# researchmm/MM-Diffusion

Hardware: AMD Instinct MI355X
Metric: denoising steps/sec (video+audio pair), 16x64x64 / 25600 (higher is better)
Workload: dtype bf16; 1 GPU; BASELINE configs[1]: Landscape base model (133.68M params), DDPM p_sample, timestep_respacing=250, per-GPU batch 4, 16x3x64x64 video + 1x25600 audio; global_batch=4, parallelism=batch-sharded x1, no in-loop collective, weights=key-seeded synthetic (mm_diffusion.synth), graph_replay=True, batch_lanes=2, finite=True, ranks_seen=1

## Files before the change

### include/mmd.h

```cpp
#ifndef MMD_H
#define MMD_H
#include <stdint.h>
#ifdef __cplusplus
extern "C" {
#endif

#define MMD_F32 0
#define MMD_BF16 1
#define MMD_OK 0
#define MMD_ERR_ARG (-1)
#define MMD_ERR_LAUNCH (-2)
#define MMD_ERR_UNSUPPORTED (-3)

int mmd_version(void);
const char* mmd_last_error(void);
int mmd_debug_install_crash_handler(void);

int mmd_graph_begin(void* stream);
int mmd_graph_end(void* stream, void** exec_out);
int mmd_graph_launch(void* exec, void* stream);
int mmd_graph_destroy(void* exec);
int mmd_stream_create(void** stream_out);
int mmd_stream_sync(void* stream);
int mmd_stream_destroy(void* stream);
int mmd_event_create(void** ev);
int mmd_event_record(void* ev, void* stream);
int mmd_stream_wait_event(void* stream, void* ev);
int mmd_event_elapsed_ms(void* ev_start, void* ev_stop, float* ms);
int mmd_event_destroy(void* ev);

int mmd_temb_fwd(const void* t, int t_kind, int N, int dim, const float* W0, const float* b0, const float* W2,
                 const float* b2, float* out_silu, float* out_raw, void* stream);

int mmd_linear_fwd(const float* x, const float* W, const float* b, float* y, int N, int K, int J, void* stream);

int64_t mmd_gn_workspace_bytes(int dtype, int C, int S, int Tn);
int mmd_gn_stats(int dtype, const void* x, int64_t ld, int C, int S, int Tn, int inner, int64_t outer_stride,
                 int64_t inner_stride, int64_t tstride, const float* gamma, const float* beta, const float* film,
                 int64_t film_ld, float eps, float* a_out, float* b_out, float* mr_out, void* workspace, void* stream);
int mmd_gn_finalize_stats(const float* rec, int64_t rec_ld, int C, int S, int Tn, const float* gamma, const float* beta,
                          const float* film, int64_t film_ld, float eps, float* a_out, float* b_out, float* mr_out, void* stream);
int mmd_gn_apply(int dtype, const void* x, int64_t ldx, void* y, int64_t ldy, int64_t rows, int C, int S, int Tn, int inner,
                 int64_t outer_stride, int64_t inner_stride, int64_t tstride, const float* a, const float* b, int act,
                 void* stream);
int mmd_add_rowbias(int dtype, void* x, int64_t ld, int64_t rows, int C, int64_t rows_per_sample, const float* e,
                    int64_t e_ld, void* stream);
int mmd_colsum_slices(int dtype, const void* dY, int64_t lddy, int S, int64_t Tn, int C, float* out, int64_t ldo, void* stream);

int mmd_conv_gemm(int dtype, const void* A, int64_t lda, const void* W, const float* bias, const void* R, int64_t ldr,
                  void* Y, int64_t ldy, int M, int Cout, int Cin, int ntaps, const int* taps, int D0, int D1, int D2, int tile,
                  void* stream);

int mmd_gn_conv1x1(int dtype, const void* A, int64_t lda, const float* gn_a, const float* gn_b, int act, int S,
                   int64_t rows_per_slice, const void* W, const float* bias, const void* R, int64_t ldr, void* Y, int64_t ldy,
                   int M, int Cout, int Cin, int tile, void* stream);

int mmd_gn_small(int dtype, const void* x, int64_t ldx, void* y, int64_t ldy, int C, int S, int Tn, int inner, int64_t outer_stride,
                 int64_t inner_stride, int64_t tstride, const float* gamma, const float* beta, float eps, int act, void* stream);

int mmd_gn_group(int dtype, const void* x, int64_t ldx, void* y, int64_t ldy, int C, int S, int Tn, int inner, int64_t outer_stride,
                 int64_t inner_stride, int64_t tstride, const float* gamma, const float* beta, const float* film, int64_t film_ld,
                 float eps, int act, float* a_out, float* b_out, float* mr_out, void* stream);

int mmd_zero(void* ptr, int64_t bytes, void* stream);

int mmd_conv_gemm_stats(int dtype, const void* A, int64_t lda, const void* W, const float* bias, const void* R, int64_t ldr,
                        void* Y, int64_t ldy, int M, int Cout, int Cin, int ntaps, const int* taps, int D0, int D1, int D2, int tile,
                        float* stats, int64_t stats_ld, void* stream);
int mmd_gn_conv1x1_stats(int dtype, const void* A, int64_t lda, const float* gn_a, const float* gn_b, int act, int S,
                         int64_t rows_per_slice, const void* W, const float* bias, const void* R, int64_t ldr, void* Y, int64_t ldy,
                         int M, int Cout, int Cin, int tile, float* stats, int64_t stats_ld, void* stream);

int mmd_gn_conv1x1_skip(int dtype, const void* h, int64_t ldh, const float* gn_a, const float* gn_b, int act, int S,
                        int64_t rows_per_slice, const void* W_out, const float* bias_out, const void* x, int64_t ldx, int K2,
                        const void* W_skip, const float* bias_skip, void* Y, int64_t ldy, int M, int Cout, int K1, float* stats,
                        int64_t stats_ld, void* stream);

// ... 184 lines not shown
```

### mm-diffusion_amd/csrc/mmd_norm.hip

```cpp
#include "mmd_common.h"

#define GN_GROUPS 32
typedef __attribute__((ext_vector_type(2))) double f64x2;

struct SliceGeom {
  int S, Tn, inner;
  int64_t outer_stride, inner_stride, tstride;
};

__device__ __forceinline__ int64_t slice_base(const SliceGeom& g, int s) {
  return (int64_t)(s / g.inner) * g.outer_stride + (int64_t)(s % g.inner) * g.inner_stride;
}
__device__ __forceinline__ int slice_of_row(const SliceGeom& g, int64_t m) {
  const int64_t o = m / g.outer_stride, rem = m % g.outer_stride;
  return (int)(o * g.inner + (rem / g.inner_stride) % g.inner);
}

template <typename T, bool ONE>
__global__ __launch_bounds__(256) void gn_partial_kernel(const char* __restrict__ x, int64_t ld, int C, SliceGeom g, int R,
                                                         double* __restrict__ part, int nchunks,
                                                         const float* __restrict__ gamma, const float* __restrict__ beta,
                                                         const float* __restrict__ film, int64_t film_ld, float eps,
                                                         float* __restrict__ a_out, float* __restrict__ b_out, float* __restrict__ mr_out) {
  constexpr int EPV = Elt<T>::EPV;
// ... 149 lines not shown
    }
    s_pa[cl][gi] = (a[0] + a[1]) + (a[2] + a[3]);
    s_pb[cl][gi] = (b[0] + b[1]) + (b[2] + b[3]);
  }
  __syncthreads();
  if (tid < GN_GROUPS) {
    double a = 0.0, b = 0.0;
    for (int k = 0; k < 32; ++k) { a += s_pa[k][tid]; b += s_pb[k][tid]; }
    const double cnt = (double)Tn * (double)cpg;
    const double dm = a / cnt;
    double var = b / cnt - dm * dm;
    if (var < 0.0) var = 0.0;
    s_mean[tid] = (float)(piv + dm);
    s_rstd[tid] = (float)(1.0 / sqrt(var + (double)eps));
    if (mr_out) {
      mr_out[((int64_t)s * GN_GROUPS + tid) * 2] = s_mean[tid];
      mr_out[((int64_t)s * GN_GROUPS + tid) * 2 + 1] = s_rstd[tid];
    }
  }
  __syncthreads();
#pragma unroll
  for (int k = 0; k < CPT; ++k) {
    const int c = tid + k * 1024;
    if (c < C) {
      const int gi = c / cpg;
      const float a = s_rstd[gi] * gm[k];
      const float b = bt[k] - s_mean[gi] * a;
      a_out[(int64_t)s * C + c] = a * fsc[k];
      b_out[(int64_t)s * C + c] = b * fsc[k] + fsh[k];
    }
  }
}

template <typename T>
__global__ __launch_bounds__(256) void gn_apply_kernel(const char* __restrict__ x, int64_t ldx, char* __restrict__ y, int64_t ldy,
                                                       int C, SliceGeom g, const float* __restrict__ a,
                                                       const float* __restrict__ b, int act, int R) {
  constexpr int EPV = Elt<T>::EPV;
  constexpr int ES = 16 / EPV;
  const int s = blockIdx.y, chunk = blockIdx.x, tid = threadIdx.x;
  const int CV = C / EPV, CVB = min(CV, 256), RPP = 256 / CVB;
  const int col0 = tid % CVB, rl = tid / CVB;
  if (rl >= RPP) return;
  for (int cp = 0; cp < CV; cp += 256) {
  const int col = col0 + cp;
  if (col >= CV) break;
  float av[EPV], bv[EPV];
#pragma unroll
  for (int e = 0; e < EPV; e += 4) {
    const f32x4 a4 = *(const f32x4*)(a + (int64_t)s * C + col * EPV + e), b4 = *(const f32x4*)(b + (int64_t)s * C + col * EPV + e);
#pragma unroll
    for (int k = 0; k < 4; ++k) { av[e + k] = a4[k]; bv[e + k] = b4[k]; }
  }
  const int64_t base = slice_base(g, s);
  const char* xp = x + (base * ldx + (int64_t)col * EPV) * ES;
  char* yp = y + (base * ldy + (int64_t)col * EPV) * ES;
  const int64_t xs = g.tstride * ldx * ES, ys = g.tstride * ldy * ES;
  const int j0 = chunk * R, j1 = min(j0 + R, g.Tn);
  for (int jb = j0 + rl; jb < j1; jb += 4 * RPP) {
    u32x4 v[4];
#pragma unroll
    for (int u = 0; u < 4; ++u) {
      const int j = jb + u * RPP;
      if (j < j1) v[u] = *(const u32x4*)(xp + (int64_t)j * xs);
    }
#pragma unroll
    for (int u = 0; u < 4; ++u) {
      const int j = jb + u * RPP;
      if (j < j1) {
        float f[EPV];
        Elt<T>::unpack(v[u], f);
#pragma unroll
        for (int e = 0; e < EPV; ++e) {
          const float w = f[e] * av[e] + bv[e];
          f[e] = act ? silu_f(w) : w;
        }
        *(u32x4*)(yp + (int64_t)j * ys) = Elt<T>::pack(f);
      }
    }
  }
  }
}

template <typename T>
__global__ __launch_bounds__(256) void gn_small_kernel(const char* __restrict__ x, int64_t ldx, char* __restrict__ y, int64_t ldy, int C,
                                                       SliceGeom g, const float* __restrict__ gamma, const float* __restrict__ beta,
                                                       float eps, int act, int SPB) {
  constexpr int EPV = Elt<T>::EPV, ES = 16 / EPV, MAXT = 16, QPV = EPV / 4;
  extern __shared__ __attribute__((aligned(16))) char smem[];
  float* sQ = (float*)smem;
  const int CV = C / EPV, NQ = C / 4, cpg = C / GN_GROUPS, qpg = cpg / 4;
  const int tid = threadIdx.x, pl = tid / CV, cv = tid - pl * CV;
  const int s = blockIdx.x * SPB + pl;
  const bool live = pl < SPB && s < g.S;
  u32x4 v[MAXT];
  const int64_t base = live ? slice_base(g, s) : 0;
  const char* xp = x + (base * ldx + (int64_t)cv * EPV) * ES;
  const int64_t xs = g.tstride * ldx * ES;
#pragma unroll
  for (int j = 0; j < MAXT; ++j)
    if (live && j < g.Tn) v[j] = *(const u32x4*)(xp + (int64_t)j * xs);
  float q[2] = {0.f, 0.f};
  if (live) {
#pragma unroll
    for (int j = 0; j < MAXT; ++j)
      if (j < g.Tn) {
        float f[EPV];
        Elt<T>::unpack(v[j], f);
#pragma unroll
// ... 103 lines not shown
  if (C <= 0 || S <= 0 || Tn <= 0) return 0;
  return (int64_t)S * cdiv(Tn, gn_rows_per_block(dtype, C, S, Tn)) * GN_GROUPS * 2 * sizeof(double);
}

extern "C" int mmd_gn_stats(int dtype, const void* x, int64_t ld, int C, int S, int Tn, int inner, int64_t outer_stride,
                            int64_t inner_stride, int64_t tstride, const float* gamma, const float* beta,
                            const float* film, int64_t film_ld, float eps, float* a_out, float* b_out, float* mr_out,
                            void* workspace, void* stream) {
  int rc = check_geom("gn_stats", dtype, C, S, Tn, inner);
  if (rc) return rc;
  MMD_REQUIRE(x && gamma && beta && a_out && b_out, "gn_stats: null pointer");
  MMD_REQUIRE(((uintptr_t)x) % 16 == 0 && ld % (dtype == MMD_BF16 ? 8 : 4) == 0, "gn_stats: x must be 16-byte aligned rows");
  SliceGeom g{S, Tn, inner, outer_stride, inner_stride, tstride};
  hipStream_t st = (hipStream_t)stream;
  const int R = gn_rows_per_block(dtype, C, S, Tn);
  const int nchunks = cdiv(Tn, R);
  if (nchunks == 1)
    return mmd_by_dtype(dtype, [&](auto t) {
      return mmd_launch<gn_partial_kernel<typename decltype(t)::type, true>>("gn_stats_one", dim3(1, S), dim3(256), 0, st, (const char*)x, ld, C, g, R,
                                                                             (double*)nullptr, 1, gamma, beta, film, film_ld, eps, a_out, b_out, mr_out);
    });
  MMD_REQUIRE(workspace && ((uintptr_t)workspace) % 16 == 0, "gn_stats: 16-byte aligned workspace required for multi-block slices");
  dim3 grid(nchunks, S);
  rc = mmd_by_dtype(dtype, [&](auto t) {
    return mmd_launch<gn_partial_kernel<typename decltype(t)::type, false>>("gn_partial", grid, dim3(256), 0, st, (const char*)x, ld, C, g, R,
                                                                            (double*)workspace, nchunks, gamma, beta, film, film_ld, eps, a_out, b_out,
                                                                            (float*)nullptr);
  });
  if (rc) return rc;
  return mmd_launch<gn_finalize_kernel>("gn_finalize", dim3(S), dim3(1024), 0, st, (const char*)x, dtype, ld, g, (const double*)workspace, nchunks, C, Tn,
                                        gamma, beta, film, film_ld, eps, a_out, b_out, mr_out);
}

__global__ __launch_bounds__(256) void gn_finalize_rec_kernel(const float* __restrict__ rec, int64_t rec_ld, int C, int S, int Tn,
                                                              const float* __restrict__ gamma, const float* __restrict__ beta,
                                                              const float* __restrict__ film, int64_t film_ld, float eps,
                                                              float* __restrict__ a_out, float* __restrict__ b_out, float* __restrict__ mr_out) {
  __shared__ double s_a[4], s_b[4];
  const int gi = blockIdx.x, s = blockIdx.y, tid = threadIdx.x;
  const int cpg = C / GN_GROUPS, qpg = cpg / 4;
  const int nrec = Tn / 64;
  const float* base = rec + ((int64_t)s * nrec * rec_ld + (int64_t)gi * qpg) * 2;
  const int total = nrec * qpg;
  const int c = gi * cpg + min(tid, cpg - 1);
  const float gv = gamma[c], bv0 = beta[c];
  float fsc = 0.f, fsh = 0.f;
  if (film) {
    fsc = film[(int64_t)s * film_ld + c];
    fsh = film[(int64_t)s * film_ld + C + c];
  }
  double a[4] = {0.0, 0.0, 0.0, 0.0}, b[4] = {0.0, 0.0, 0.0, 0.0};
  for (int i = tid; i < total; i += 1024) {
#pragma unroll
    for (int u = 0; u < 4; ++u) {
      const int k = i + 256 * u;
      const int kk = min(k, total - 1);
      const int r = kk / qpg, cq = kk - r * qpg;
      const float2 v = *(const float2*)(base + ((int64_t)r * rec_ld + cq) * 2);
      const double m = k < total ? 1.0 : 0.0;
      a[u] += m * (double)v.x;
      b[u] += m * (double)v.y;
    }
  }
  double ta = (a[0] + a[1]) + (a[2] + a[3]), tb = (b[0] + b[1]) + (b[2] + b[3]);
  ta = wave_sum_d(ta);
  tb = wave_sum_d(tb);
  if ((tid & 63) == 0) { s_a[tid >> 6] = ta; s_b[tid >> 6] = tb; }
  __syncthreads();
  if (tid < cpg) {
    const double sa = (s_a[0] + s_a[1]) + (s_a[2] + s_a[3]), sb = (s_b[0] + s_b[1]) + (s_b[2] + s_b[3]);
    const double cnt = (double)Tn * (double)cpg;
    const double mean = sa / cnt;
    double var = sb / cnt - mean * mean;
    if (var < 0.0) var = 0.0;
    const float mean_f = (float)mean, rstd_f = (float)(1.0 / sqrt(var + (double)eps));
    if (mr_out && tid == 0) {
      mr_out[((int64_t)s * GN_GROUPS + gi) * 2] = mean_f;
      mr_out[((int64_t)s * GN_GROUPS + gi) * 2 + 1] = rstd_f;
    }
    float av = rstd_f * gv;
    float bv = bv0 - mean_f * av;
    if (film) {
      const float sc = 1.f + fsc;
      av *= sc;
      bv = bv * sc + fsh;
    }
    a_out[(int64_t)s * C + c] = av;
    b_out[(int64_t)s * C + c] = bv;
  }
}

extern "C" int mmd_gn_finalize_stats(const float* rec, int64_t rec_ld, int C, int S, int Tn, const float* gamma, const float* beta,
                                     const float* film, int64_t film_ld, float eps, float* a_out, float* b_out, float* mr_out,
                                     void* stream) {
  MMD_REQUIRE(rec && gamma && beta && a_out && b_out, "gn_finalize_stats: null pointer");
  MMD_REQUIRE(C > 0 && C % (4 * GN_GROUPS) == 0 && C / GN_GROUPS <= 256 && rec_ld >= C / 4,
              "gn_finalize_stats: channel count %d (groups of whole quads: a multiple of 128; ld %ld quads)", C, (long)rec_ld);
  MMD_REQUIRE(S > 0 && Tn > 0 && Tn % 64 == 0, "gn_finalize_stats: slices must be multiples of 64 rows (S=%d Tn=%d)", S, Tn);
  return mmd_launch<gn_finalize_rec_kernel>("gn_finalize_stats", dim3(GN_GROUPS, S), dim3(256), 0, (hipStream_t)stream, rec, rec_ld, C, S, Tn, gamma, beta,
                                            film, film_ld, eps, a_out, b_out, mr_out);
}

template <typename T>
__global__ __launch_bounds__(256) void gn_group_kernel(const char* __restrict__ x, int64_t ldx, char* __restrict__ y, int64_t ldy, int C,
                                                       SliceGeom g, const float* __restrict__ gamma, const float* __restrict__ beta,
                                                       const float* __restrict__ film, int64_t film_ld, float eps, int act,
                                                       float* __restrict__ a_out, float* __restrict__ b_out, float* __restrict__ mr_out) {
  constexpr int ES = sizeof(T), MAXI = 16;
  __shared__ float s_red[2][4];
  __shared__ float s_ab[2][64];
  const int gi = blockIdx.x, s = blockIdx.y, tid = threadIdx.x;
  const int cpg = C / GN_GROUPS, qpg = cpg / 4, items = g.Tn * qpg;
  const int64_t base = slice_base(g, s);
  const char* xg = x + (int64_t)gi * cpg * ES;
  float f[MAXI][4];
#pragma unroll
  for (int j = 0; j < MAXI; ++j) {
    const int i = tid + 256 * j;
    if (i < items) {
      const int r = i / qpg, k = i - r * qpg;
      const char* q = xg + ((base + (int64_t)r * g.tstride) * ldx + 4 * k) * ES;
      if constexpr (ES == 2) {
        const u32x2 v = *(const u32x2*)q;
        f[j][0] = __uint_as_float(v[0] << 16); f[j][1] = __uint_as_float(v[0] & 0xffff0000u);
        f[j][2] = __uint_as_float(v[1] << 16); f[j][3] = __uint_as_float(v[1] & 0xffff0000u);
      } else {
        const f32x4 v = *(const f32x4*)q;
        f[j][0] = v[0]; f[j][1] = v[1]; f[j][2] = v[2]; f[j][3] = v[3];
      }
    } else {
      f[j][0] = f[j][1] = f[j][2] = f[j][3] = 0.f;
    }
// ... 70 lines not shown
  if (rc) return rc;
  MMD_REQUIRE(x && gamma && beta && (y || a_out), "gn_group: null pointer (needs y or a_out / b_out)");
  MMD_REQUIRE((a_out == nullptr) == (b_out == nullptr), "gn_group: a_out and b_out come together");
  MMD_REQUIRE(C % 128 == 0 && C <= 2048, "gn_group: groups of whole channel quads, at most 2048 channels (C = %d)", C);
  MMD_REQUIRE((int64_t)Tn * (C / 128) <= 4096, "gn_group: a (group, slice) of %d rows x %d channels does not fit one block's registers", Tn, C / 32);
  const int eb = dtype == MMD_BF16 ? 2 : 4;
  MMD_REQUIRE(((uintptr_t)x) % 16 == 0 && ldx % 4 == 0 && (!y || (((uintptr_t)y) % 16 == 0 && ldy % 4 == 0)), "gn_group: rows must be aligned to channel quads");
  (void)eb;
  SliceGeom g{S, Tn, inner, outer_stride, inner_stride, tstride};
  return mmd_by_dtype(dtype, [&](auto t) {
    return mmd_launch<gn_group_kernel<typename decltype(t)::type>>("gn_group", dim3(GN_GROUPS, S), dim3(256), 0, (hipStream_t)stream, (const char*)x, ldx,
                                                                   (char*)y, ldy, C, g, gamma, beta, film, film_ld, eps, act, a_out, b_out, mr_out);
  });
}

extern "C" int mmd_gn_apply(int dtype, const void* x, int64_t ldx, void* y, int64_t ldy, int64_t rows, int C, int S, int Tn,
                            int inner, int64_t outer_stride, int64_t inner_stride, int64_t tstride, const float* a,
                            const float* b, int act, void* stream) {
  int rc = check_geom("gn_apply", dtype, C, S, Tn, inner);
  if (rc) return rc;
  MMD_REQUIRE(x && y && a && b && rows > 0, "gn_apply: null pointer / empty");
  SliceGeom g{S, Tn, inner, outer_stride, inner_stride, tstride};
  MMD_REQUIRE(rows == (int64_t)S * Tn, "gn_apply: rows %ld != S*Tn (%d x %d): the slices must tile the rows", (long)rows, S, Tn);
  const int rpp = max(1, 256 / (C / (dtype == MMD_BF16 ? 8 : 4)));
  int R = 4 * rpp;
  while ((int64_t)S * cdiv(Tn, R) > 4096 && R < 4096) R *= 2;
  dim3 grid(cdiv(Tn, R), S);
  hipStream_t st = (hipStream_t)stream;
  return mmd_by_dtype(dtype, [&](auto t) {
    return mmd_launch<gn_apply_kernel<typename decltype(t)::type>>("gn_apply", grid, dim3(256), 0, st, (const char*)x, ldx, (char*)y, ldy, C, g, a, b, act, R);
  });
}

extern "C" int mmd_add_rowbias(int dtype, void* x, int64_t ld, int64_t rows, int C, int64_t rows_per_sample, const float* e,
                               int64_t e_ld, void* stream) {
  MMD_REQUIRE(dtype == MMD_BF16 || dtype == MMD_F32, "add_rowbias: bad dtype");
  MMD_REQUIRE(x && e && rows > 0 && C % 8 == 0, "add_rowbias: bad argument");
  const int64_t total = rows * (C / (dtype == MMD_BF16 ? 8 : 4));
  const int grid = (int)min((int64_t)4096, (total + 255) / 256);
  hipStream_t st = (hipStream_t)stream;
  return mmd_by_dtype(dtype, [&](auto t) {
    return mmd_launch<add_rowbias_kernel<typename decltype(t)::type>>("add_rowbias", dim3(grid), dim3(256), 0, st, (char*)x, ld, rows, C, rows_per_sample, e, e_ld);
  });
}

extern "C" int mmd_gn_small(int dtype, const void* x, int64_t ldx, void* y, int64_t ldy, int C, int S, int Tn, int inner,
                            int64_t outer_stride, int64_t inner_stride, int64_t tstride, const float* gamma, const float* beta,
                            float eps, int act, void* stream) {
  int rc = check_geom("gn_small", dtype, C, S, Tn, inner);
  if (rc) return rc;
  MMD_REQUIRE(C / (dtype == MMD_BF16 ? 8 : 4) <= 256, "gn_small: rows of at most 256 16-byte vectors (C = %d)", C);
  MMD_REQUIRE(x && y && gamma && beta, "gn_small: null pointer");
  MMD_REQUIRE(Tn <= 16 && (C / GN_GROUPS) % 4 == 0, "gn_small: slices of at most 16 rows, groups of whole channel quads (got Tn=%d C=%d)", Tn, C);
  SliceGeom g{S, Tn, inner, outer_stride, inner_stride, tstride};
  const int cv = C / (dtype == MMD_BF16 ? 8 : 4);
  MMD_REQUIRE(cv <= 256, "gn_small: %d channels is too wide", C);
  const int spb = 256 / cv;
  const size_t lds = (size_t)spb * (C / 4) * sizeof(float);
  return mmd_by_dtype(dtype, [&](auto t) {
    return mmd_launch<gn_small_kernel<typename decltype(t)::type>>("gn_small", dim3(cdiv(S, spb)), dim3(256), lds, (hipStream_t)stream, (const char*)x, ldx,
                                                                   (char*)y, ldy, C, g, gamma, beta, eps, act, spb);
  });
}
```

### mm-diffusion_amd/mm_diffusion/_hip.py

```python
import ctypes as C
import gc
import os

import torch

_HERE = os.path.dirname(os.path.abspath(__file__))
LIB_PATH = os.environ.get("MMD_LIB") or os.path.join(os.path.dirname(_HERE), "lib", "libmmd.so")

F32, BF16 = 0, 1
_lib = None

i32, i64, f32, vp = C.c_int, C.c_int64, C.c_float, C.c_void_p


_PROTOS = {
    "mmd_version": (C.c_int, []),
    "mmd_last_error": (C.c_char_p, []),
    "mmd_debug_install_crash_handler": (i32, []),
    "mmd_graph_begin": (i32, [vp]),
    "mmd_graph_end": (i32, [vp, C.POINTER(vp)]),
    "mmd_graph_launch": (i32, [vp, vp]),
    "mmd_graph_destroy": (i32, [vp]),
    "mmd_stream_create": (i32, [C.POINTER(vp)]),
    "mmd_stream_sync": (i32, [vp]),
    "mmd_stream_destroy": (i32, [vp]),
    "mmd_event_create": (i32, [C.POINTER(vp)]),
    "mmd_event_record": (i32, [vp, vp]),
    "mmd_stream_wait_event": (i32, [vp, vp]),
    "mmd_event_elapsed_ms": (i32, [vp, vp, C.POINTER(f32)]),
    "mmd_event_destroy": (i32, [vp]),
    "mmd_temb_fwd": (i32, [vp, i32, i32, i32, vp, vp, vp, vp, vp, vp, vp]),
    "mmd_linear_fwd": (i32, [vp, vp, vp, vp, i32, i32, i32, vp]),
    "mmd_gn_workspace_bytes": (i64, [i32, i32, i32, i32]),
    "mmd_gn_stats": (i32, [i32, vp, i64, i32, i32, i32, i32, i64, i64, i64, vp, vp, vp, i64, f32, vp, vp, vp, vp, vp]),
    "mmd_gn_small": (i32, [i32, vp, i64, vp, i64, i32, i32, i32, i32, i64, i64, i64, vp, vp, f32, i32, vp]),
    "mmd_gn_group": (i32, [i32, vp, i64, vp, i64, i32, i32, i32, i32, i64, i64, i64, vp, vp, vp, i64, f32, i32, vp, vp, vp, vp]),
    "mmd_gn_apply": (i32, [i32, vp, i64, vp, i64, i64, i32, i32, i32, i32, i64, i64, i64, vp, vp, i32, vp]),
    "mmd_add_rowbias": (i32, [i32, vp, i64, i64, i32, i64, vp, i64, vp]),
    "mmd_colsum_slices": (i32, [i32, vp, i64, i32, i64, i32, vp, i64, vp]),
    "mmd_conv_gemm": (i32, [i32, vp, i64, vp, vp, vp, i64, vp, i64, i32, i32, i32, i32, C.POINTER(i32), i32, i32, i32, i32, vp]),
    "mmd_gn_conv1x1": (i32, [i32, vp, i64, vp, vp, i32, i32, i64, vp, vp, vp, i64, vp, i64, i32, i32, i32, i32, vp]),
    "mmd_conv_gemm_stats": (i32, [i32, vp, i64, vp, vp, vp, i64, vp, i64, i32, i32, i32, i32, C.POINTER(i32), i32, i32, i32, i32, vp, i64, vp]),
    "mmd_gn_conv1x1_stats": (i32, [i32, vp, i64, vp, vp, i32, i32, i64, vp, vp, vp, i64, vp, i64, i32, i32, i32, i32, vp, i64, vp]),
    "mmd_gn_conv1x1_skip": (i32, [i32, vp, i64, vp, vp, i32, i32, i64, vp, vp, vp, i64, i32, vp, vp, vp, i64, i32, i32, i32, vp, i64, vp]),
    "mmd_res_tail": (i32, [vp, i64, vp, vp, i32, vp, vp, vp, i64, vp, vp, vp, i64, i32, i32, i32, i32, i32, vp, i64, vp]),
    "mmd_gn_conv_gemm": (i32, [i32, vp, i64, vp, vp, i32, i32, i64, vp, vp, vp, i64, vp, i64, i32, i32, i32, i32, C.POINTER(i32), i32, i32, i32, i32, vp]),
    "mmd_tconv_weight_bytes": (i64, [i32, i32]),
    "mmd_tconv_pack": (i32, [vp, vp, i32, i32, vp]),
    "mmd_tconv": (i32, [vp, i64, vp, vp, vp, i64, i32, i32, i32, i32, i32, vp, i64, vp]),
    "mmd_aconv": (i32, [vp, i64, vp, vp, vp, vp, i32, vp, i64, i32, i32, i32, i32, i32, vp, i64, vp]),
    "mmd_tattn_weight_bytes": (i64, [i32, i32]),
    "mmd_tattn_pack": (i32, [vp, vp, vp, vp, i32, vp]),
    "mmd_tattn_block": (i32, [vp, i64, vp, i64, vp, i64, vp, vp, vp, vp, vp, vp, f32, vp, i64, i32, i32, i32, i32, i32, vp, i64, vp]),
    "mmd_vconv2d1d_weight_bytes": (i64, [i32]),
    "mmd_vconv2d1d_pack": (i32, [vp, vp, vp, i32, i32, vp]),
    "mmd_vconv2d1d": (i32, [vp, i64, vp, vp, i32, i32, i64, vp, vp, vp, vp, i64, i32, i32, i32, i32, i32, i32, vp, i64, vp]),
    "mmd_zero": (i32, [vp, i64, vp]),
    "mmd_gn_finalize_stats": (i32, [vp, i64, i32, i32, i32, vp, vp, vp, i64, f32, vp, vp, vp, vp]),
    "mmd_attn_fwd": (i32, [i32, vp, i64, i32, vp, i64, i32, i32, vp, i64, i32, i32, i32, i32, i64, i32, i64, i32, i32, vp, i32, vp]),
    "mmd_attn_small_fwd": (i32, [i32, vp, i64, vp, i64, i32, i32, i32, i32, i32, i64, i64, i64, vp]),
    "mmd_resample": (i32, [i32, vp, i64, vp, i64, i32, i32, i32, i32, i32, i32, i32, f32, vp]),
    "mmd_resample_stats": (i32, [vp, i64, vp, i64, i32, i32, i32, i32, i32, i32, i32, vp, i64, vp]),
    "mmd_copy2d": (i32, [vp, i64, vp, i64, i64, i64, vp]),
    "mmd_stem_conv": (i32, [i32, vp, vp, vp, vp, i64, i32, i32, i32, i32, i32, i32, i32, C.POINTER(i32), vp]),
    "mmd_head_conv": (i32, [i32, vp, i64, vp, vp, vp, i32, i32, i32, i32, i32, i32, i32, C.POINTER(i32), vp]),
    "mmd_head_gemm_weight_bytes": (i64, [i32]),
    "mmd_head_gemm_workspace_bytes": (i64, [i64, i32, i32]),
    "mmd_head_gemm": (i32, [vp, i64, i64, i32, vp, vp, i32, i64, i32, vp, vp, i32, vp]),
    "mmd_head_gather": (i32, [vp, vp, vp, i32, i32, i32, i32, i32, i32, C.POINTER(i32), vp]),
    "mmd_ddpm_update": (i32, [vp, vp, vp, vp, vp, vp, vp, vp, vp, i32, i32, i32, i32, i32, i32, vp]),
# ... 232 lines not shown
```

### mm-diffusion_amd/mm_diffusion/engine.py

```python
import os
from types import SimpleNamespace

import torch

from . import _hip as H
from . import ops
from .ops import Geom


_EMB_ON_AUDIO_STREAM = ops._flag("MMD_EMB_AUX")
_POOL_NOREUSE = os.environ.get("MMD_POOL_NOREUSE") == "1"
_UP_LOWRES = ops._flag("MMD_UP_LOWRES")
_CROSS_SERIAL = ops._flag("MMD_CROSS_SERIAL")
_RESAMPLE_STATS = ops._flag("MMD_RESAMPLE_STATS")
_SKIP_FUSE = ops._flag("MMD_SKIP_FUSE")
_TAIL_STREAM = ops._TAIL_STREAM


class _Pool:

    def __init__(self, device):
        self.device = device
        self.free = []
        self.all = []

    def get(self, nbytes):
        nbytes = (int(nbytes) + 255) // 256 * 256
        best = None
        for i, raw in enumerate(self.free):
            sz = raw.numel()
            if sz >= nbytes and sz <= 2 * nbytes + 65536 and (best is None or sz < self.free[best].numel()):
                best = i
        if best is not None:
            return self.free.pop(best)
        raw = torch.empty(nbytes, dtype=torch.uint8, device=self.device)
        self.all.append(raw)
        return raw

    def put(self, raw):
        if not _POOL_NOREUSE:
            self.free.append(raw)

    def total_bytes(self):
        return sum(r.numel() for r in self.all)


class UNetEngine:
    def __init__(self, model, N, dtype, device):
        if not torch.cuda.is_available():
# ... 101 lines not shown
        cache = self.model.__dict__.setdefault("_wcache", {})
        if cache.get("sig") != self._sig:
            cache.clear()
            cache["sig"] = self._sig
        k = (kind, key, self.dtype if kind == "gemm" else None, str(self.device))
        t = cache.get(k)
        if t is None:
            t = cache[k] = make()
        self.keep.append(t)
        return t

    def _f32(self, key):
        return self._packed("f32", key, lambda: self.params[key].detach().float().contiguous())

    def _gemm_w(self, key):
        return self._packed("gemm", key, lambda: ops.pack_conv_weight(self.params[key].detach().float(), self.dtype))

    def _edge_w(self, key):
        return self._packed("edge", key, lambda: ops.pack_edge_weight(self.params[key].detach()))

    def _temporal(self, Hh):
        if ops.HALO_CANDIDATE:
            return dict(taps=ops.TAPS_TEMPORAL_D1, dims=(self.N, self.F, Hh * Hh))
        return dict(taps=ops.TAPS_TEMPORAL, dims=(self.F, Hh * Hh, 1))

    def _gn(self, x, prefix, geom, act, film=None, out=None):
        C = x.shape[1]
        if film is None and self._gn_small and ops.gn_small_ok(x, geom):
            y = self._alloc(x.shape[0], C) if out is None else out
            return ops.gn_small(x, self._f32(prefix + ".GroupNorm.weight"), self._f32(prefix + ".GroupNorm.bias"), geom, act=act, out=y)
        if ops.gn_group_ok(x, geom) and self._rec_ready(x, geom) is None:
            y = self._alloc(x.shape[0], C) if out is None else out
            return ops.gn_group(x, self._f32(prefix + ".GroupNorm.weight"), self._f32(prefix + ".GroupNorm.bias"), geom, film=film, out=y, act=act)
        a, b = self._gn_affine(x, prefix, geom, film)
        y = self._alloc(x.shape[0], C) if out is None else out
        ops.gn_apply(x, a, b, geom, act=act, out=y)
        self._release(a, b)
        return y

    def _gn_affine(self, x, prefix, geom, film):
        C = x.shape[1]
        a = self._alloc(geom.S, C, torch.float32)
        b = self._alloc(geom.S, C, torch.float32)
        gamma, beta = self._f32(prefix + ".GroupNorm.weight"), self._f32(prefix + ".GroupNorm.bias")
        rec = self._rec_ready(x, geom)
        if rec is not None:
            ops.gn_finalize_stats(rec, gamma, beta, geom, film=film, a=a, b=b)
        elif ops.gn_group_ok(x, geom):
            ops.gn_group(x, gamma, beta, geom, film=film, a=a, b=b)
        else:
            ws = self._alloc(ops.gn_workspace_bytes(x, geom) // 8, 1, torch.float64)
            ops.gn_stats(x, gamma, beta, geom, film=film, a=a, b=b, ws=ws)
            self._release(ws)
        return a, b

    def _gn_pw(self, x, gn_prefix, geom, act, wkey, bkey, film=None, residual=None, out=None):
        C = x.shape[1]
        Cout = self.params[wkey].shape[0]
        will_emit = True if (out is not None and self._rec_slice(out)[0] is not None) else None
        if not ops.gn_fusable(geom, C, Cout, x, will_emit, act):
            n1 = self._gn(x, gn_prefix, geom, act, film=film)
            y = self._pw(n1, wkey, bkey, residual=residual, out=out)
            self._release(n1)
            return y
        a, b = self._gn_affine(x, gn_prefix, geom, film)
        y = self._alloc(x.shape[0], Cout) if out is None else out
# ... 477 lines not shown
```

### mm-diffusion_amd/mm_diffusion/ops.py

```python
import contextlib
import os

import torch

from . import _hip as H

GN_EPS = 1e-5

_recorder = None
_keep = None


class recording:
    def __init__(self, plan, keep=None):
        self.plan, self.keep = plan, keep

    def __enter__(self):
        global _recorder, _keep
        self._prev, _recorder = (_recorder, _keep), self.plan
        _keep = self.keep
        return self.plan

    def __exit__(self, *a):
        global _recorder, _keep
# ... 119 lines not shown
def gn_stats(x, gamma, beta, geom: Geom, film=None, a=None, b=None, ws=None, mr=None):
    _chk2d(x)
    C = x.shape[1]
    a = alloc(geom.S, C, dtype=torch.float32, device=x.device) if a is None else a
    b = alloc(geom.S, C, dtype=torch.float32, device=x.device) if b is None else b
    ws = gn_workspace(x, geom) if ws is None else ws
    _dispatch("mmd_gn_stats", H.dt_of(x), x.data_ptr(), x.stride(0), C, *geom.args(), gamma.data_ptr(), beta.data_ptr(),
           H.ptr(film), 0 if film is None else film.stride(0), GN_EPS, a.data_ptr(), b.data_ptr(), H.ptr(mr), ws.data_ptr(),
           meta=(f"gn_stats[S={geom.S},Tn={geom.Tn},C={C}]", 0, geom.S * geom.Tn * C * x.element_size()))
    return a, b


def gn_finalize_stats(rec, gamma, beta, geom: Geom, film=None, a=None, b=None, mr=None):
    C = rec.shape[1] * 4
    if C % 128:
        raise H.MMDError("gn_finalize_stats: the normalised channels must be a multiple of 128 (groups of whole quads)")
    if not geom.covers(rec.shape[0] * 64) or geom.Tn % 64:
        raise H.MMDError("gn_finalize_stats: needs contiguous slices that are multiples of 64 rows")
    a = alloc(geom.S, C, dtype=torch.float32, device=rec.device) if a is None else a
    b = alloc(geom.S, C, dtype=torch.float32, device=rec.device) if b is None else b
    _dispatch("mmd_gn_finalize_stats", rec.data_ptr(), rec.stride(0) // 2, C, geom.S, geom.Tn, gamma.data_ptr(), beta.data_ptr(),
              H.ptr(film), 0 if film is None else film.stride(0), GN_EPS, a.data_ptr(), b.data_ptr(), H.ptr(mr),
              meta=(f"gn_finalize_stats[S={geom.S},Tn={geom.Tn},C={C}]", 0, rec.shape[0] * C * 8))
    return a, b


def gn_apply(x, a, b, geom: Geom, act=True, out=None):
    _chk2d(x)
    out = alloc(x.shape, dtype=x.dtype, device=x.device) if out is None else out
    _chk2d(out)
    _dispatch("mmd_gn_apply", H.dt_of(x), x.data_ptr(), x.stride(0), out.data_ptr(), out.stride(0), x.shape[0], x.shape[1],
           *geom.args(), a.data_ptr(), b.data_ptr(), 1 if act else 0,
           meta=("gn_apply", 0, 2 * x.shape[0] * x.shape[1] * x.element_size()))
    return out


def zero(t):
    H.require_cuda(t)
    _dispatch("mmd_zero", t.data_ptr(), t.numel() * t.element_size(), meta=("zero", 0, t.numel() * t.element_size()))
    return t


def gn_small_ok(x, geom: Geom):
    return geom.Tn <= 16 and x.shape[1] % 128 == 0 and x.shape[1] // (8 if x.element_size() == 2 else 4) <= 256


def gn_small(x, gamma, beta, geom: Geom, act=False, out=None):
    _chk2d(x)
    out = alloc(x.shape, dtype=x.dtype, device=x.device) if out is None else out
    _chk2d(out)
    _dispatch("mmd_gn_small", H.dt_of(x), x.data_ptr(), x.stride(0), out.data_ptr(), out.stride(0), x.shape[1], *geom.args(), gamma.data_ptr(),
              beta.data_ptr(), GN_EPS, 1 if act else 0, meta=(f"gn_small[S={geom.S},Tn={geom.Tn},C={x.shape[1]}]", 0, 2 * x.shape[0] * x.shape[1] * x.element_size()))
    return out


_GN_GROUP = _flag("MMD_GN_GROUP")


def gn_group_ok(x, geom: Geom):
    C = x.shape[1]
    return _GN_GROUP and C % 128 == 0 and C <= 2048 and geom.Tn * (C // 128) <= 4096 and x.stride(0) % 4 == 0


def gn_group(x, gamma, beta, geom: Geom, film=None, a=None, b=None, out=None, act=False, mr=None):
    _chk2d(x)
    C = x.shape[1]
# ... 1175 lines not shown
```

Baseline: 380.0 pair-steps/s.

## Fuse GroupNorm record finalize into apply kernel for small slices

Adds a gn_rec_apply kernel that reduces the precomputed per-64-row records into group mean/rstd inside each apply block, builds the affine in shared memory, and normalizes+SiLU the tile. This replaces the separate finalize-stats launch plus gn_apply launch when slices are small enough. It also swaps the integer division in the record fold for a magic-number multiply-high, and prefetches the first input rows before the stats reduction. Each block redoes the group reduction, so redundant work grows with the number of row chunks, which is why it is gated to small slices.

New measurement: 380.2 pair-steps/s, median of 3. No clear change (+0.0%).

```diff
diff --git a/include/mmd.h b/include/mmd.h
--- a/include/mmd.h
+++ b/include/mmd.h
@@ -43,6 +43,9 @@
 int mmd_gn_apply(int dtype, const void* x, int64_t ldx, void* y, int64_t ldy, int64_t rows, int C, int S, int Tn, int inner,
                  int64_t outer_stride, int64_t inner_stride, int64_t tstride, const float* a, const float* b, int act,
                  void* stream);
+int mmd_gn_rec_apply(int dtype, const void* x, int64_t ldx, void* y, int64_t ldy, const float* rec, int64_t rec_ld, int C, int S, int Tn,
+                     const float* gamma, const float* beta, const float* film, int64_t film_ld, float eps, int act, float* a_out,
+                     float* b_out, void* stream);
 int mmd_add_rowbias(int dtype, void* x, int64_t ld, int64_t rows, int C, int64_t rows_per_sample, const float* e,
                     int64_t e_ld, void* stream);
 int mmd_colsum_slices(int dtype, const void* dY, int64_t lddy, int S, int64_t Tn, int C, float* out, int64_t ldo, void* stream);
diff --git a/mm-diffusion_amd/csrc/mmd_norm.hip b/mm-diffusion_amd/csrc/mmd_norm.hip
--- a/mm-diffusion_amd/csrc/mmd_norm.hip
+++ b/mm-diffusion_amd/csrc/mmd_norm.hip
@@ -205,6 +205,11 @@
   }
 }
 
+__device__ __forceinline__ float gn_apply_elem(float f, float a, float b, int act) {
+  const float w = f * a + b;
+  return act ? silu_f(w) : w;
+}
+
 template <typename T>
 __global__ __launch_bounds__(256) void gn_apply_kernel(const char* __restrict__ x, int64_t ldx, char* __restrict__ y, int64_t ldy,
                                                        int C, SliceGeom g, const float* __restrict__ a,
@@ -244,10 +249,7 @@
         float f[EPV];
         Elt<T>::unpack(v[u], f);
 #pragma unroll
-        for (int e = 0; e < EPV; ++e) {
-          const float w = f[e] * av[e] + bv[e];
-          f[e] = act ? silu_f(w) : w;
-        }
+        for (int e = 0; e < EPV; ++e) f[e] = gn_apply_elem(f[e], av[e], bv[e], act);
         *(u32x4*)(yp + (int64_t)j * ys) = Elt<T>::pack(f);
       }
     }
@@ -417,7 +419,67 @@
                                         gamma, beta, film, film_ld, eps, a_out, b_out, mr_out);
 }
 
-__global__ __launch_bounds__(256) void gn_finalize_rec_kernel(const float* __restrict__ rec, int64_t rec_ld, int C, int S, int Tn,
+static uint32_t gn_qmagic(int qpg) { return qpg <= 1 ? 0u : (uint32_t)((((uint64_t)1 << 32) + (uint64_t)qpg - 1) / (uint64_t)qpg); }
+
+template <int P>
+__device__ __forceinline__ void gn_rec_thread_sums(const float* __restrict__ base, int64_t rec_ld, int qpg, uint32_t qmagic, int total,
+                                                   int tid0, double (&ta)[P], double (&tb)[P]) {
+  double a[P][4], b[P][4];
+#pragma unroll
+  for (int p = 0; p < P; ++p)
+#pragma unroll
+    for (int u = 0; u < 4; ++u) a[p][u] = b[p][u] = 0.0;
+  for (int i0 = 0; i0 < total; i0 += 1024) {
+    float2 v[P][4];
+#pragma unroll
+    for (int p = 0; p < P; ++p)
+#pragma unroll
+      for (int u = 0; u < 4; ++u) {
+        const int kk = min(i0 + tid0 + 64 * p + 256 * u, total - 1);
+        const int r = qmagic ? (int)__umulhi((uint32_t)kk, qmagic) : kk, cq = kk - r * qpg;
+        v[p][u] = *(const float2*)(base + ((int64_t)r * rec_ld + cq) * 2);
+      }
+#pragma unroll
+    for (int p = 0; p < P; ++p)
+      if (i0 + tid0 + 64 * p < total) {
+#pragma unroll
+        for (int u = 0; u < 4; ++u) {
+          const double m = i0 + tid0 + 64 * p + 256 * u < total ? 1.0 : 0.0;
+          a[p][u] += m * (double)v[p][u].x;
+          b[p][u] += m * (double)v[p][u].y;
+        }
+      }
+  }
+#pragma unroll
+  for (int p = 0; p < P; ++p) {
+    ta[p] = (a[p][0] + a[p][1]) + (a[p][2] + a[p][3]);
+    tb[p] = (b[p][0] + b[p][1]) + (b[p][2] + b[p][3]);
+  }
+}
+
+__device__ __forceinline__ void gn_rec_mean_rstd(const double (&wa)[4], const double (&wb)[4], int Tn, int cpg, float eps, float& mean_f,
+                                                 float& rstd_f) {
+  const double sa = (wa[0] + wa[1]) + (wa[2] + wa[3]), sb = (wb[0] + wb[1]) + (wb[2] + wb[3]);
+  const double cnt = (double)Tn * (double)cpg;
+  const double mean = sa / cnt;
+  double var = sb / cnt - mean * mean;
+  if (var < 0.0) var = 0.0;
+  mean_f = (float)mean;
+  rstd_f = (float)(1.0 / sqrt(var + (double)eps));
+}
+
+__device__ __forceinline__ void gn_rec_affine(float mean_f, float rstd_f, float gv, float bv0, bool has_film, float fsc, float fsh, float& av,
+                                              float& bv) {
+  av = rstd_f * gv;
+  bv = bv0 - mean_f * av;
+  if (has_film) {
+    const float sc = 1.f + fsc;
+    av *= sc;
+    bv = bv * sc + fsh;
+  }
+}
+
+__global__ __launch_bounds__(256) void gn_finalize_rec_kernel(const float* __restrict__ rec, int64_t rec_ld, int C, int S, int Tn, uint32_t qmagic,
                                                               const float* __restrict__ gamma, const float* __restrict__ beta,
                                                               const float* __restrict__ film, int64_t film_ld, float eps,
                                                               float* __restrict__ a_out, float* __restrict__ b_out, float* __restrict__ mr_out) {
@@ -434,44 +496,113 @@
     fsc = film[(int64_t)s * film_ld + c];
     fsh = film[(int64_t)s * film_ld + C + c];
   }
-  double a[4] = {0.0, 0.0, 0.0, 0.0}, b[4] = {0.0, 0.0, 0.0, 0.0};
-  for (int i = tid; i < total; i += 1024) {
-#pragma unroll
-    for (int u = 0; u < 4; ++u) {
-      const int k = i + 256 * u;
-      const int kk = min(k, total - 1);
-      const int r = kk / qpg, cq = kk - r * qpg;
-      const float2 v = *(const float2*)(base + ((int64_t)r * rec_ld + cq) * 2);
-      const double m = k < total ? 1.0 : 0.0;
-      a[u] += m * (double)v.x;
-      b[u] += m * (double)v.y;
-    }
-  }
-  double ta = (a[0] + a[1]) + (a[2] + a[3]), tb = (b[0] + b[1]) + (b[2] + b[3]);
-  ta = wave_sum_d(ta);
-  tb = wave_sum_d(tb);
-  if ((tid & 63) == 0) { s_a[tid >> 6] = ta; s_b[tid >> 6] = tb; }
+  double ta[1], tb[1];
+  gn_rec_thread_sums<1>(base, rec_ld, qpg, qmagic, total, tid, ta, tb);
+  ta[0] = wave_sum_d(ta[0]);
+  tb[0] = wave_sum_d(tb[0]);
+  if ((tid & 63) == 0) { s_a[tid >> 6] = ta[0]; s_b[tid >> 6] = tb[0]; }
   __syncthreads();
   if (tid < cpg) {
-    const double sa = (s_a[0] + s_a[1]) + (s_a[2] + s_a[3]), sb = (s_b[0] + s_b[1]) + (s_b[2] + s_b[3]);
-    const double cnt = (double)Tn * (double)cpg;
-    const double mean = sa / cnt;
-    double var = sb / cnt - mean * mean;
-    if (var < 0.0) var = 0.0;
-    const float mean_f = (float)mean, rstd_f = (float)(1.0 / sqrt(var + (double)eps));
+    const double wa[4] = {s_a[0], s_a[1], s_a[2], s_a[3]}, wb[4] = {s_b[0], s_b[1], s_b[2], s_b[3]};
+    float mean_f, rstd_f, av, bv;
+    gn_rec_mean_rstd(wa, wb, Tn, cpg, eps, mean_f, rstd_f);
     if (mr_out && tid == 0) {
       mr_out[((int64_t)s * GN_GROUPS + gi) * 2] = mean_f;
       mr_out[((int64_t)s * GN_GROUPS + gi) * 2 + 1] = rstd_f;
     }
-    float av = rstd_f * gv;
-    float bv = bv0 - mean_f * av;
-    if (film) {
-      const float sc = 1.f + fsc;
-      av *= sc;
-      bv = bv * sc + fsh;
-    }
+    gn_rec_affine(mean_f, rstd_f, gv, bv0, film != nullptr, fsc, fsh, av, bv);
     a_out[(int64_t)s * C + c] = av;
     b_out[(int64_t)s * C + c] = bv;
+  }
+}
+
+template <typename T>
+__global__ __launch_bounds__(256) void gn_rec_apply_kernel(const char* __restrict__ x, int64_t ldx, char* __restrict__ y, int64_t ldy,
+                                                           const float* __restrict__ rec, int64_t rec_ld, int C, int Tn, uint32_t qmagic,
+                                                           const float* __restrict__ gamma, const float* __restrict__ beta,
+                                                           const float* __restrict__ film, int64_t film_ld, float eps, int act, int R,
+                                                           float* __restrict__ a_out, float* __restrict__ b_out) {
+  constexpr int EPV = Elt<T>::EPV;
+  constexpr int ES = 16 / EPV;
+  __shared__ __attribute__((aligned(16))) float s_av[256], s_bv[256];
+  const int chunk = blockIdx.x, cb = blockIdx.y, s = blockIdx.z, tid = threadIdx.x;
+  const int lane = tid & 63, w = tid >> 6;
+  const int cpg = C / GN_GROUPS, qpg = cpg / 4;
+  const int nrec = Tn / 64;
+  const int total = nrec * qpg;
+  const int CVB = 4 * cpg / EPV, RPP = 256 / CVB;
+  const int col = tid % CVB, rl = tid / CVB;
+  const bool live = rl < RPP;
+  const int64_t c0 = (int64_t)cb * 4 * cpg + (int64_t)col * EPV;
+  const char* xp = x + ((int64_t)s * Tn * ldx + c0) * ES;
+  char* yp = y + ((int64_t)s * Tn * ldy + c0) * ES;
+  const int64_t xs = ldx * ES, ys = ldy * ES;
+  const int j0 = chunk * R, j1 = min(j0 + R, Tn);
+  int jb = j0 + rl;
+  u32x4 v[4];
+#pragma unroll
+  for (int u = 0; u < 4; ++u) {
+    const int j = jb + u * RPP;
+    if (live && j < j1) v[u] = *(const u32x4*)(xp + (int64_t)j * xs);
+  }
+  {
+    const int gi = cb * 4 + w;
+    const float* base = rec + ((int64_t)s * nrec * rec_ld + (int64_t)gi * qpg) * 2;
+    const int c = gi * cpg + min(lane, cpg - 1);
+    const float gv = gamma[c], bv0 = beta[c];
+    float fsc = 0.f, fsh = 0.f;
+    if (film) {
+      fsc = film[(int64_t)s * film_ld + c];
+      fsh = film[(int64_t)s * film_ld + C + c];
+    }
+    double wa[4], wb[4];
+    gn_rec_thread_sums<4>(base, rec_ld, qpg, qmagic, total, lane, wa, wb);
+#pragma unroll
+    for (int p = 0; p < 4; ++p)
+      if (64 * p < total) {
+        wa[p] = wave_sum_d(wa[p]);
+        wb[p] = wave_sum_d(wb[p]);
+      }
+    if (lane < cpg) {
+      float mean_f, rstd_f, av, bv;
+      gn_rec_mean_rstd(wa, wb, Tn, cpg, eps, mean_f, rstd_f);
+      gn_rec_affine(mean_f, rstd_f, gv, bv0, film != nullptr, fsc, fsh, av, bv);
+      s_av[w * cpg + lane] = av;
+      s_bv[w * cpg + lane] = bv;
+      if (a_out && chunk == 0) {
+        a_out[(int64_t)s * C + c] = av;
+        b_out[(int64_t)s * C + c] = bv;
+      }
+    }
+  }
+  __syncthreads();
+  if (!live) return;
+  float av[EPV], bv[EPV];
+#pragma unroll
+  for (int e = 0; e < EPV; e += 4) {
+    const f32x4 a4 = *(const f32x4*)(s_av + col * EPV + e), b4 = *(const f32x4*)(s_bv + col * EPV + e);
+#pragma unroll
+    for (int k = 0; k < 4; ++k) { av[e + k] = a4[k]; bv[e + k] = b4[k]; }
+  }
+  while (true) {
+#pragma unroll
+    for (int u = 0; u < 4; ++u) {
+      const int j = jb + u * RPP;
+      if (j < j1) {
+        float f[EPV];
+        Elt<T>::unpack(v[u], f);
+#pragma unroll
+        for (int e = 0; e < EPV; ++e) f[e] = gn_apply_elem(f[e], av[e], bv[e], act);
+        *(u32x4*)(yp + (int64_t)j * ys) = Elt<T>::pack(f);
+      }
+    }
+    jb += 4 * RPP;
+    if (jb >= j1) break;
+#pragma unroll
+    for (int u = 0; u < 4; ++u) {
+      const int j = jb + u * RPP;
+      if (j < j1) v[u] = *(const u32x4*)(xp + (int64_t)j * xs);
+    }
   }
 }
 
@@ -482,7 +613,8 @@
   MMD_REQUIRE(C > 0 && C % (4 * GN_GROUPS) == 0 && C / GN_GROUPS <= 256 && rec_ld >= C / 4,
               "gn_finalize_stats: channel count %d (groups of whole quads: a multiple of 128; ld %ld quads)", C, (long)rec_ld);
   MMD_REQUIRE(S > 0 && Tn > 0 && Tn % 64 == 0, "gn_finalize_stats: slices must be multiples of 64 rows (S=%d Tn=%d)", S, Tn);
-  return mmd_launch<gn_finalize_rec_kernel>("gn_finalize_stats", dim3(GN_GROUPS, S), dim3(256), 0, (hipStream_t)stream, rec, rec_ld, C, S, Tn, gamma, beta,
+  MMD_REQUIRE((int64_t)(Tn / 64) * (C / 128) < ((int64_t)1 << 25), "gn_finalize_stats: %d x %d is more records per group than the fold indexes", Tn, C);
+  return mmd_launch<gn_finalize_rec_kernel>("gn_finalize_stats", dim3(GN_GROUPS, S), dim3(256), 0, (hipStream_t)stream, rec, rec_ld, C, S, Tn, gn_qmagic(C / (4 * GN_GROUPS)), gamma, beta,
                                             film, film_ld, eps, a_out, b_out, mr_out);
 }
 
@@ -619,6 +751,31 @@
   });
 }
 
+extern "C" int mmd_gn_rec_apply(int dtype, const void* x, int64_t ldx, void* y, int64_t ldy, const float* rec, int64_t rec_ld, int C, int S,
+                                int Tn, const float* gamma, const float* beta, const float* film, int64_t film_ld, float eps, int act,
+                                float* a_out, float* b_out, void* stream) {
+  MMD_REQUIRE(dtype == MMD_BF16 || dtype == MMD_F32, "gn_rec_apply: bad dtype %d", dtype);
+  MMD_REQUIRE(x && y && rec && gamma && beta, "gn_rec_apply: null pointer");
+  MMD_REQUIRE((a_out == nullptr) == (b_out == nullptr), "gn_rec_apply: a_out and b_out come together");
+  MMD_REQUIRE(C > 0 && C % (4 * GN_GROUPS) == 0 && C <= 2048 && rec_ld >= C / 4,
+              "gn_rec_apply: channel count %d (groups of whole quads: a multiple of 128, at most 2048; ld %ld quads)", C, (long)rec_ld);
+  MMD_REQUIRE(S > 0 && S <= 65535 && Tn > 0 && Tn % 64 == 0, "gn_rec_apply: slices must be multiples of 64 rows (S=%d Tn=%d)", S, Tn);
+  MMD_REQUIRE((int64_t)(Tn / 64) * (C / 128) < ((int64_t)1 << 25), "gn_rec_apply: %d x %d is more records per group than the fold indexes", Tn, C);
+  const int epv = dtype == MMD_BF16 ? 8 : 4;
+  MMD_REQUIRE(((uintptr_t)x) % 16 == 0 && ((uintptr_t)y) % 16 == 0 && ldx % epv == 0 && ldy % epv == 0 && ldx >= C && ldy >= C,
+              "gn_rec_apply: x and y must be 16-byte aligned rows of at least C elements");
+  MMD_REQUIRE(((uintptr_t)rec) % 8 == 0 && (!film || film_ld >= 2 * (int64_t)C), "gn_rec_apply: unaligned records / FiLM rows shorter than 2 C");
+  const int cvb = C / 8 / epv, rpp = 256 / cvb;
+  int R = 4 * rpp;
+  while ((int64_t)S * (GN_GROUPS / 4) * cdiv(Tn, R) > 1024 && R < 4096) R *= 2;
+  dim3 grid(cdiv(Tn, R), GN_GROUPS / 4, S);
+  return mmd_by_dtype(dtype, [&](auto t) {
+    return mmd_launch<gn_rec_apply_kernel<typename decltype(t)::type>>("gn_rec_apply", grid, dim3(256), 0, (hipStream_t)stream, (const char*)x, ldx,
+                                                                       (char*)y, ldy, rec, rec_ld, C, Tn, gn_qmagic(C / (4 * GN_GROUPS)), gamma, beta, film, film_ld, eps, act, R,
+                                                                       a_out, b_out);
+  });
+}
+
 extern "C" int mmd_add_rowbias(int dtype, void* x, int64_t ld, int64_t rows, int C, int64_t rows_per_sample, const float* e,
                                int64_t e_ld, void* stream) {
   MMD_REQUIRE(dtype == MMD_BF16 || dtype == MMD_F32, "add_rowbias: bad dtype");
diff --git a/mm-diffusion_amd/mm_diffusion/_hip.py b/mm-diffusion_amd/mm_diffusion/_hip.py
--- a/mm-diffusion_amd/mm_diffusion/_hip.py
+++ b/mm-diffusion_amd/mm_diffusion/_hip.py
@@ -36,6 +36,7 @@
     "mmd_gn_small": (i32, [i32, vp, i64, vp, i64, i32, i32, i32, i32, i64, i64, i64, vp, vp, f32, i32, vp]),
     "mmd_gn_group": (i32, [i32, vp, i64, vp, i64, i32, i32, i32, i32, i64, i64, i64, vp, vp, vp, i64, f32, i32, vp, vp, vp, vp]),
     "mmd_gn_apply": (i32, [i32, vp, i64, vp, i64, i64, i32, i32, i32, i32, i64, i64, i64, vp, vp, i32, vp]),
+    "mmd_gn_rec_apply": (i32, [i32, vp, i64, vp, i64, vp, i64, i32, i32, i32, vp, vp, vp, i64, f32, i32, vp, vp, vp]),
     "mmd_add_rowbias": (i32, [i32, vp, i64, i64, i32, i64, vp, i64, vp]),
     "mmd_colsum_slices": (i32, [i32, vp, i64, i32, i64, i32, vp, i64, vp]),
     "mmd_conv_gemm": (i32, [i32, vp, i64, vp, vp, vp, i64, vp, i64, i32, i32, i32, i32, C.POINTER(i32), i32, i32, i32, i32, vp]),
diff --git a/mm-diffusion_amd/mm_diffusion/engine.py b/mm-diffusion_amd/mm_diffusion/engine.py
--- a/mm-diffusion_amd/mm_diffusion/engine.py
+++ b/mm-diffusion_amd/mm_diffusion/engine.py
@@ -15,6 +15,7 @@
 _RESAMPLE_STATS = ops._flag("MMD_RESAMPLE_STATS")
 _SKIP_FUSE = ops._flag("MMD_SKIP_FUSE")
 _TAIL_STREAM = ops._TAIL_STREAM
+_GN_REC_APPLY = ops._GN_REC_APPLY != "0"
 
 
 class _Pool:
@@ -182,6 +183,11 @@
         if ops.gn_group_ok(x, geom) and self._rec_ready(x, geom) is None:
             y = self._alloc(x.shape[0], C) if out is None else out
             return ops.gn_group(x, self._f32(prefix + ".GroupNorm.weight"), self._f32(prefix + ".GroupNorm.bias"), geom, film=film, out=y, act=act)
+        rec = self._rec_ready(x, geom) if _GN_REC_APPLY else None
+        if rec is not None and ops.gn_rec_apply_ok(x, geom, out) and ops.gn_rec_apply_pays(x, geom):
+            y = self._alloc(x.shape[0], C) if out is None else out
+            return ops.gn_rec_apply(x, rec, self._f32(prefix + ".GroupNorm.weight"), self._f32(prefix + ".GroupNorm.bias"), geom, film=film,
+                                    act=act, out=y)
         a, b = self._gn_affine(x, prefix, geom, film)
         y = self._alloc(x.shape[0], C) if out is None else out
         ops.gn_apply(x, a, b, geom, act=act, out=y)
diff --git a/mm-diffusion_amd/mm_diffusion/ops.py b/mm-diffusion_amd/mm_diffusion/ops.py
--- a/mm-diffusion_amd/mm_diffusion/ops.py
+++ b/mm-diffusion_amd/mm_diffusion/ops.py
@@ -175,6 +175,50 @@
     _dispatch("mmd_gn_apply", H.dt_of(x), x.data_ptr(), x.stride(0), out.data_ptr(), out.stride(0), x.shape[0], x.shape[1],
            *geom.args(), a.data_ptr(), b.data_ptr(), 1 if act else 0,
            meta=("gn_apply", 0, 2 * x.shape[0] * x.shape[1] * x.element_size()))
+    return out
+
+
+_GN_REC_APPLY = os.environ.get("MMD_GN_REC_APPLY", "1")
+
+
+def gn_rec_apply_ok(x, geom: Geom, out=None):
+    if x.dim() != 2 or x.stride(1) != 1 or x.dtype not in (torch.bfloat16, torch.float32):
+        return False
+    C, epv = x.shape[1], 16 // x.element_size()
+    if C % 128 or not 128 <= C <= 2048 or not geom.covers(x.shape[0]) or geom.Tn % 64 or geom.S > 65535:
+        return False
+    ts = (x,) if out is None else (x, out)
+    if out is not None and (out.dim() != 2 or out.shape != x.shape or out.dtype != x.dtype):
+        return False
+    return not any(t.stride(1) != 1 or t.stride(0) % epv or t.stride(0) < C or t.data_ptr() % 16 for t in ts)
+
+
+_GN_REC_APPLY_MAX_SLICE = 1600 * 768
+
+
+def gn_rec_apply_pays(x, geom: Geom):
+    if _GN_REC_APPLY == "all":
+        return True
+    return _GN_REC_APPLY != "0" and geom.Tn * x.shape[1] <= _GN_REC_APPLY_MAX_SLICE
+
+
+def gn_rec_apply(x, rec, gamma, beta, geom: Geom, film=None, act=True, out=None, a=None, b=None):
+    _chk2d(x)
+    C = x.shape[1]
+    if rec.shape[1] * 4 != C or rec.shape[0] * 64 != x.shape[0]:
+        raise H.MMDError(f"gn_rec_apply: records {tuple(rec.shape)} do not cover x {tuple(x.shape)} (one per 64 rows and channel quad)")
+    if (a is None) != (b is None):
+        raise H.MMDError("gn_rec_apply: a and b come together")
+    out = alloc(x.shape, dtype=x.dtype, device=x.device) if out is None else out
+    _chk2d(out)
+    if not gn_rec_apply_ok(x, geom, out):
+        raise H.MMDError(f"gn_rec_apply: x {tuple(x.shape)} strides {x.stride()} / out strides {out.stride()} / S={geom.S} Tn={geom.Tn}: needs "
+                         "C % 128 == 0, contiguous slices of whole 64-row records and 16-byte aligned rows")
+    es = x.element_size()
+    _dispatch("mmd_gn_rec_apply", H.dt_of(x), x.data_ptr(), x.stride(0), out.data_ptr(), out.stride(0), rec.data_ptr(), rec.stride(0) // 2, C,
+              geom.S, geom.Tn, gamma.data_ptr(), beta.data_ptr(), H.ptr(film), 0 if film is None else film.stride(0), GN_EPS,
+              1 if act else 0, H.ptr(a), H.ptr(b),
+              meta=(f"gn_rec_apply[S={geom.S},Tn={geom.Tn},C={C}]", 0, 2 * x.shape[0] * C * es + rec.shape[0] * C * 2))
     return out
 
 
```
